# MiloszKrajewski/lz4net

Measured on AMD Instinct MI355X. Metric: uncompressed GB/s, batched 64KiB-block encode+decode: value = decode (known output size) per step over the whole resident batch; fast encode and LZ4HC encode of the same data in roofline_encode / roofline_hc, higher is better.
Workload: dtype u8

## Files before the change

lz4net_amd/csrc/lz4hip_decode_lane4.hpp:

```cpp
#pragma once
#include "lz4hip_common.hpp"
#include <type_traits>

#ifndef LZ4HIP_ITERATION_HOOK
#define LZ4HIP_ITERATION_HOOK(lane) ((void)0)
#endif
#ifndef LZ4HIP_STAT
#define LZ4HIP_STAT(slot, cond) ((void)0)
#endif
#ifdef LZ4HIP_SECTION_MARKERS
#define LZ4HIP_SECTION(name) asm volatile("; @@SECTION " name)
#else
#define LZ4HIP_SECTION(name) ((void)0)
#endif

namespace lz4hip {

#ifndef LZ4HIP_DEC4_FLUSH_RECS
#define LZ4HIP_DEC4_FLUSH_RECS 0
#endif
#ifndef LZ4HIP_DEC4_DUAL_STORE
#define LZ4HIP_DEC4_DUAL_STORE 2
#endif
constexpr unsigned lane4_lds_bytes(int ring_bytes) { return 64u * (unsigned)ring_bytes + 16u * 32u; }

struct NoNext {
    static constexpr bool kPersistent = false;
    LZ4HIP_DEVICE bool operator()(int, const uint8_t*&, int&, uint8_t*&, int&) const { return false; }
};

enum L4Kind { kK4None = 0, kK4Near = 1, kK4Far = 2, kK4Lit = 3, kK4Zero = 4 };
enum L4Flag { kF4Final = 1, kF4Err = 2, kF4Header = 4 };

template <bool KNOWN, int R, int P, int FU, int FS, int FE = 1, int IE = 1, int POL = 0, class NEXT = NoNext, int WAVES = 1>
LZ4HIP_DEVICE int lane4_decode_block(unsigned char* lds, int lane, bool active, const uint8_t* src, int iend,
                                     uint8_t* dst, int oend, NEXT next = NEXT(), int wave = 0)
{
    static_assert(WAVES == 1 || WAVES == 4, "one or four wavefronts per workgroup");
    constexpr uint32_t kRow = 256u * (uint32_t)WAVES;
    static_assert(R >= 128 && R % 16 == 0 && R <= 1008, "ring: a multiple of 16 bytes, 128 .. 1008");
    static_assert(P == 32 || P == 64, "input piece: 32 or 64 bytes");
    static_assert(FU == 64 || (FU == 128 && R >= 192), "flush unit: 64 bytes, or 128 with a ring of at least 192");
    static_assert(FS == 1 || FS == 2, "one or two flush store instructions per iteration");
    static_assert(FE == 1 || FE == 2, "the flush runs in every iteration or in every second one");
    static_assert(IE == 1 || (IE == 2 && FE == 2), "input requests in every iteration, or alternating with the flush");
    constexpr int RW = R / 4;
    constexpr bool RPOW2 = (RW & (RW - 1)) == 0;
    constexpr uint32_t kRingBytes = (uint32_t)RW * kRow;
    constexpr uint32_t kLdsBytes = lane4_lds_bytes(R) * (uint32_t)WAVES;
    constexpr bool LS = (POL & 16) != 0;
    constexpr int kDual = (POL & 32) ? 0 : (LZ4HIP_DEC4_DUAL_STORE);
    static_assert(!LS || P == 32, "sector input feeds 32-byte pieces");
    constexpr int SK = LS ? 64 : P;
    constexpr int NW = 4 + P / 4, NL = LS ? 4 : P / 16;
    constexpr int HPR = FU / 16, RECS_PER_STORE = 64 / HPR;
    constexpr int kFlushRecs = (LZ4HIP_DEC4_FLUSH_RECS) ? (LZ4HIP_DEC4_FLUSH_RECS) : FS * RECS_PER_STORE;
    constexpr bool kLineNoWrap = R % 64 == 0;
    constexpr int kNearMax = R - 20;
    unsigned char* const frec_base = lds + kRingBytes + (uint32_t)wave * 256u;
    auto frec = [&](int i) -> Aligned16* {
        if (kFlushRecs <= 16) return (Aligned16*)(frec_base + (uint32_t)i * 16u);
        return (Aligned16*)(frec_base + (uint32_t)(i >> 4) * kRow + (uint32_t)(i & 15) * 16u);
    };
    const uint32_t lane4 = (uint32_t)(wave * 64 + lane) << 2;

    auto ring_add = [](uint32_t a, uint32_t rows256) -> uint32_t {
        const uint32_t t = a + rows256;
        if (RPOW2) return t & (kRingBytes - 1u);
        const uint32_t u = t - kRingBytes;
        return u < t ? u : t;
    };
#define L4_RING(a) (*(uint32_t*)(lds + (a)))
#define L4_PHASE_SEL(p_) wv::alignbyte(0x07060504u, 0x03020100u, (uint32_t)(p_) & 3u)

    int skew = 0, in_total = 0;
    uint64_t src_al = 0;
    uint32_t out_limit = 0;
    int ip = 0;
    uint32_t W[NW];
    wv::u32x4 L[NL];
    int wb = -16;
    int lvalid = 0;
    int pend_a = 0, pend_b = 0;
    int op = 0, fl = 0;
    uint32_t oa = lane4;
    int kind = kK4None, rem = 0, off = 8;
    int gready = 0;
    int pv = 0, p_ll = 0, p_st = 0, p_ml = 0, p_off = 0, p_flags = 0, p_res = 0;
    uint32_t p_l0 = 0, p_l1 = 0, p_l2 = 0;
    int hdr = 0;
    uint32_t token = 0;
    int final_seen = 0, final_run = 0, result = 0, done = 0;
    int exhausted = 0;
    wv::u32x4 fa = { 0, 0, 0, 0 }, fb = { 0, 0, 0, 0 };
#if defined(LZ4HIP_DEC4_BALLAST_VALU) || defined(LZ4HIP_DEC4_BALLAST_LDS)
    uint32_t ballast = 0;
#endif
#pragma unroll
    for (int j = 0; j < NW; j++) W[j] = 0;
#pragma unroll
    for (int j = 0; j < NL; j++) L[j] = wv::u32x4{ 0, 0, 0, 0 };
    auto start_block = [&](bool act) {
        skew = (int)((uint64_t)src & (uint64_t)(SK - 1));
        src_al = (uint64_t)src - (uint64_t)skew;
        in_total = iend > 0 ? (int)(((int64_t)skew + iend + P - 1) & ~(int64_t)(P - 1)) : 0;
        out_limit = oend > kLastLiterals ? (uint32_t)(oend - kLastLiterals) : 0u;
        ip = 0; wb = -16 - P; lvalid = 0; pend_a = 0; pend_b = 0; op = 0; fl = 0; oa = lane4;
        kind = kK4None; rem = 0; off = 8; gready = 0;
        pv = 0; p_ll = 0; p_st = 0; p_ml = 0; p_off = 0; p_flags = 0; p_res = 0; hdr = 0; token = 0;
        final_seen = 0; final_run = 0; result = 0; done = 0;
        if (!act || (!KNOWN && iend == 0)) { done = 1; final_seen = 1; }
    };
    start_block(active);

#define L4_STORE2(OFF_, v_) do { const uint32_t w_ = (v_); wv::lds_store_drop<OFF_>(lds, kLdsBytes, oa, w_); wv::lds_store_drop<OFF_>(lds, kLdsBytes, ob_, w_); } while (0)
#define L4_APPEND(d0_, d1_, d2_, d3_, n_, FOUR_)                                                         \
    do {                                                                                                \
        const uint32_t sb_ = (uint32_t)op & 3u;                                                         \
        const uint32_t s_ = wv::alignbyte(0x08070605u, 0x04030201u, sb_ ^ 3u);                          \
        wv::lds_mskor(&L4_RING(oa), 0xFFFFFFFFu << (8u * sb_), wv::perm(d0_, 0u, s_));                  \
        if (kDual) {                                                                                    \
                                                    \
            const uint32_t ob_ = oa - kRingBytes;                                                       \
            const uint32_t w1_ = wv::perm(d1_, d0_, s_), w2_ = wv::perm(d2_, d1_, s_);                  \
            if (kDual == 2) {                                         \
                wv::lds_store2_rows_drop<1 * WAVES, 2 * WAVES>(lds, kLdsBytes, oa, w1_, w2_);           \
                wv::lds_store2_rows_drop<1 * WAVES, 2 * WAVES>(lds, kLdsBytes, ob_, w1_, w2_);          \
                if (FOUR_) {                                                                            \
                    const uint32_t w3_ = wv::perm(d3_, d2_, s_), w4_ = wv::perm(0u, d3_, s_);           \
                    wv::lds_store2_rows_drop<3 * WAVES, 4 * WAVES>(lds, kLdsBytes, oa, w3_, w4_);       \
                    wv::lds_store2_rows_drop<3 * WAVES, 4 * WAVES>(lds, kLdsBytes, ob_, w3_, w4_);      \
                } else {                                                                                \
                    L4_STORE2(3 * kRow, wv::perm(0u, d2_, s_));                                         \
                }                                                                                       \
            } else {                                                                                    \
                L4_STORE2(kRow, w1_);                                                                   \
                L4_STORE2(2 * kRow, w2_);                                                               \
                if (FOUR_) {                                                                            \
                    L4_STORE2(3 * kRow, wv::perm(d3_, d2_, s_));                                        \
                    L4_STORE2(4 * kRow, wv::perm(0u, d3_, s_));                                         \
                } else {                                                                                \
                    L4_STORE2(3 * kRow, wv::perm(0u, d2_, s_));                                         \
                }                                                                                       \
            }                                                                                           \
        } else {                                                                                        \
            const uint32_t a1_ = ring_add(oa, kRow), a2_ = ring_add(oa, 2 * kRow), a3_ = ring_add(oa, 3 * kRow); \
            L4_RING(a1_) = wv::perm(d1_, d0_, s_);                                                      \
            L4_RING(a2_) = wv::perm(d2_, d1_, s_);                                                      \
            if (FOUR_) {                                                                                \
                L4_RING(a3_) = wv::perm(d3_, d2_, s_);                                                  \
                L4_RING(ring_add(oa, 4 * kRow)) = wv::perm(0u, d3_, s_);                                \
            } else {                                                                                    \
                L4_RING(a3_) = wv::perm(0u, d2_, s_);                                                   \
            }                                                                                           \
        }                                                                                               \
        oa = ring_add(oa, (((sb_ + (uint32_t)(n_)) << 6) & 0x700u) * (uint32_t)WAVES);                  \
        op += (n_);                                                                                     \
    } while (0)

    auto iteration = [&](auto flush_tag, wv::u32x4& ldF, wv::u32x4& usF, int& ld_pend, int& us_pend) __attribute__((always_inline)) -> bool {
        constexpr bool FLUSH = decltype(flush_tag)::value;
        constexpr bool INPUT = IE == 1 || !FLUSH;
        constexpr int kVm = (FLUSH ? FS : 0) + 1 + (INPUT ? NL : 0);
        LZ4HIP_ITERATION_HOOK(lane);
        LZ4HIP_SECTION("T1a window refill");
        int d = ip + skew - wb;
        {
            const bool no_more = wb + 16 + P >= in_total;
            const bool cross = (d >= P) & ((lvalid != 0) | no_more);
            const wv::mask_t cm = wv::cond(d >= P) & (wv::cond(lvalid != 0) | wv::cond(no_more));
#pragma unroll
            for (int j = 0; j < 4; j++) W[j] = wv::sel(cm, W[P / 4 + j], W[j]);
            if constexpr (LS) {
                const bool hi_half = ((wb + 16 + P) & 32) != 0;
                const wv::mask_t hm = wv::cond(((wb + 16 + P) & 32) != 0);
#pragma unroll
                for (int j = 0; j < 2; j++) {
                    W[4 + 4 * j] = wv::sel(cm, wv::sel(hm, L[2 + j].x, L[j].x), W[4 + 4 * j]); W[5 + 4 * j] = wv::sel(cm, wv::sel(hm, L[2 + j].y, L[j].y), W[5 + 4 * j]);
                    W[6 + 4 * j] = wv::sel(cm, wv::sel(hm, L[2 + j].z, L[j].z), W[6 + 4 * j]); W[7 + 4 * j] = wv::sel(cm, wv::sel(hm, L[2 + j].w, L[j].w), W[7 + 4 * j]);
                }
                lvalid = (cross & hi_half) ? 0 : lvalid;
            } else {
#pragma unroll
                for (int j = 0; j < NL; j++) {
                    W[4 + 4 * j] = wv::sel(cm, L[j].x, W[4 + 4 * j]); W[5 + 4 * j] = wv::sel(cm, L[j].y, W[5 + 4 * j]);
                    W[6 + 4 * j] = wv::sel(cm, L[j].z, W[6 + 4 * j]); W[7 + 4 * j] = wv::sel(cm, L[j].w, W[7 + 4 * j]);
                }
                lvalid = cross ? 0 : lvalid;
            }
            wb += cross ? P : 0;
            d -= cross ? P : 0;
        }
        LZ4HIP_SECTION("T1b cursor view (select tree + rotation)");
        const bool staged16 = d < P;
        LZ4HIP_STAT(0, true); LZ4HIP_STAT(1, done == 0); LZ4HIP_STAT(2, (done == 0) & !staged16);
        uint32_t x0, x1, x2, x3;
        {
            const uint32_t k = (uint32_t)d >> 2;
            uint32_t t[NW];
#pragma unroll
            for (int j = 0; j < NW; j++) t[j] = W[j];
            int n = NW;
#pragma unroll
            for (int sh = P / 8; sh >= 1; sh >>= 1) {
                const wv::mask_t m = wv::cond((k & (uint32_t)sh) != 0u);
                n -= sh;
#pragma unroll
                for (int j = 0; j < NW; j++)
                    if (j < n) t[j] = wv::sel(m, t[j + sh], t[j]);
            }
            const uint32_t sx = L4_PHASE_SEL(d);
            x0 = wv::perm(t[1], t[0], sx); x1 = wv::perm(t[2], t[1], sx); x2 = wv::perm(t[3], t[2], sx); x3 = wv::perm(t[4], t[3], sx);
        }
        LZ4HIP_SECTION("T1c near-match source rows");
        uint32_t v0, v1, v2, v3;
        {
            const uint32_t offn = kind == kK4Near ? (uint32_t)off : 4u;
            const uint32_t back = (((offn + 3u - ((uint32_t)op & 3u)) << 6) & ~0xFFu) * (uint32_t)WAVES;
            uint32_t sa;
            if (RPOW2) sa = (oa - back) & (kRingBytes - 1u);
            else { const uint32_t t = oa - back, u = t + kRingBytes; sa = u < t ? u : t; }
            const uint32_t r0 = L4_RING(sa), r1 = L4_RING(ring_add(sa, kRow)), r2 = L4_RING(ring_add(sa, 2 * kRow)),
                           r3 = L4_RING(ring_add(sa, 3 * kRow)), r4 = L4_RING(ring_add(sa, 4 * kRow));
            const uint32_t sr = L4_PHASE_SEL((uint32_t)op - offn);
            v0 = wv::perm(r1, r0, sr); v1 = wv::perm(r2, r1, sr); v2 = wv::perm(r3, r2, sr); v3 = wv::perm(r4, r3, sr);
        }

        LZ4HIP_SECTION("T2 cooperative flush");
        if constexpr (FLUSH) {
            const bool need = (done == 0) & (op - fl >= FU);
            const uint64_t needy = wv::ballot(need);
            const int cnt_all = wv::popc64(needy);
            const bool go = cnt_all != 0;
            int cnt = 0;
            bool mine = false;
            if (go) {
                cnt = cnt_all < kFlushRecs ? cnt_all : kFlushRecs;
                const int frank = wv::rank_below(needy);
                mine = need & (frank < kFlushRecs);
                if (mine) {
                    const uint64_t dp = (uint64_t)dst;
                    *frec(frank) = Aligned16{ { ring_add(oa, kRingBytes - ((((uint32_t)(op - fl)) << 6) & ~0xFFu) * (uint32_t)WAVES), (uint32_t)fl, (uint32_t)dp, (uint32_t)(dp >> 32) } };
                }
                wv::mem_sync();
            }
            const int sub = lane % HPR;
#pragma unroll
            for (int base = 0; base < FS * RECS_PER_STORE; base += RECS_PER_STORE) {
                const int idx = base + lane / HPR;
                const bool act = idx < cnt;
                const wv::mask_t act_m = wv::cond(idx < cnt);
                uint64_t g = 0;
                uint32_t q0 = 0, q1 = 0, q2 = 0, q3 = 0;
                if (act) {
                    const Aligned16 r = *frec(idx);
                    g = ((uint64_t)r.w[2] | ((uint64_t)r.w[3] << 32)) + (uint64_t)(r.w[1] + 16u * (uint32_t)sub);
                    const uint32_t b0 = ring_add(r.w[0], 4u * kRow * (uint32_t)sub);
                    if (kLineNoWrap) { q0 = L4_RING(b0); q1 = L4_RING(b0 + kRow); q2 = L4_RING(b0 + 2 * kRow); q3 = L4_RING(b0 + 3 * kRow); }
                    else { q0 = L4_RING(b0); q1 = L4_RING(ring_add(b0, kRow)); q2 = L4_RING(ring_add(b0, 2 * kRow)); q3 = L4_RING(ring_add(b0, 3 * kRow)); }
                }
                wv::vm_store16_mask(act_m, g, q0, q1, q2, q3);
            }
            LZ4HIP_STAT(3, need); LZ4HIP_STAT(4, need & !mine);
            if (go) {
                wv::mem_sync();
                fl += mine ? FU : 0;
            }
        }
        LZ4HIP_SECTION("T3 chunk size");
        const bool room = op - fl <= R - 46;
        const bool near = kind == kK4Near, lit = kind == kK4Lit;
        const bool can = room & (rem > 0) & !((kind == kK4Far) & (gready == 0)) & !(lit & !staged16);
        const int stride = (near & (off < 16)) ? off : 16;
        int n = can ? (rem < stride ? rem : stride) : 0;
        n = ((kind == kK4Zero) & (n > 8)) ? 8 : n;
        LZ4HIP_STAT(5, (done == 0) & (rem > 0)); LZ4HIP_STAT(6, (done == 0) & (rem > 0) & (n == 0)); LZ4HIP_STAT(7, (done == 0) & (rem > 0) & !room);
        LZ4HIP_STAT(8, (done == 0) & (rem > 0) & (kind == kK4Far) & (gready == 0)); LZ4HIP_STAT(9, (done == 0) & (rem > n));
        const int rem_after = rem - n;
        const int op_end = op + rem;

        LZ4HIP_SECTION("T4 parse ahead");
        const bool may_parse = (pv == 0) & (final_seen == 0) & !(lit & (rem > 0)) & staged16;
        LZ4HIP_STAT(10, may_parse); LZ4HIP_STAT(11, (done == 0) & (pv != 0));
        if (may_parse) {
            const uint32_t tok = hdr ? token : (x0 & 255u);
            const uint32_t t4 = tok >> 4, b1 = (x0 >> 8) & 255u, mlc = tok & 15u;
            const bool e1 = (hdr == 0) & (t4 == 15u), e2 = mlc == 15u;
            const int ll = hdr ? 0 : (int)t4 + (e1 ? (int)b1 : 0);
            const bool in_win = (hdr != 0) | (t4 <= 11u);
            const int o = hdr ? 0 : 1 + (int)t4;
            uint32_t ot;
            {
                const uint32_t q = (uint32_t)o >> 2;
                const wv::mask_t m1 = wv::cond((q & 1u) != 0u), m2 = wv::cond((q & 2u) != 0u);
                const uint32_t lo = wv::sel(m2, wv::sel(m1, x3, x2), wv::sel(m1, x1, x0));
                const uint32_t hi = wv::sel(m2, x3, wv::sel(m1, x2, x1));
                ot = wv::alignbyte(hi, lo, (uint32_t)o & 3u);
            }
            const int vo = (int)(ot & 0xFFFFu);
            const uint32_t extb = (ot >> 16) & 255u;
            const int ml = (int)mlc + kMinMatch + (e2 ? (int)extb : 0);
            const int lit_end = op_end + ll;
            const int p_after = ip + o + 2;
            bool trap = (ip + 16 > iend) | (e1 & (b1 == 255u)) | (ip + 1 + (e1 ? 1 : 0) + ll > iend);
            trap |= in_win & ((e2 & (extb == 255u)) | (vo > lit_end) | ((uint32_t)lit_end + (uint32_t)ml > out_limit));
            if (KNOWN) trap |= (hdr == 0) & (lit_end > oend - 8);
            else       trap |= ((hdr == 0) & ((lit_end > oend - kMfLimit) | (ip + 1 + (e1 ? 1 : 0) + ll > iend - 8))) | (in_win & e2 & !(p_after < iend - (kLastLiterals + 1)));
            p_l0 = wv::alignbyte(x1, x0, 1); p_l1 = wv::alignbyte(x2, x1, 1); p_l2 = wv::alignbyte(x3, x2, 1);
            token = tok;
            p_ll = in_win ? ll : 0;
            p_st = in_win ? 0 : ll;
            p_ml = in_win ? ml : 0;
            p_off = vo;
            p_flags = in_win ? 0 : (int)kF4Header;
            const int ip_fast = in_win ? p_after + (e2 ? 1 : 0) : ip + 1 + (e1 ? 1 : 0);
            if (trap) {
                LZ4HIP_SECTION("T4x byte-wise parser (trap)");
                int err = 0, pos = ip;
                if (!hdr) {
                    const uint32_t tk = ip < iend ? src[ip] : 0u;
                    int l = (int)(tk >> 4);
                    pos = ip + 1;
                    if (l == 15) {
                        uint32_t b = 255;
                        if (KNOWN) { do { b = pos < iend ? src[pos] : 0u; pos++; l += (int)b; if (l > (1 << 30)) { err = -pos; l = 0; break; } } while (b == 255); }
                        else       { while (pos < iend && b == 255) { b = src[pos]; pos++; l += (int)b; l = l > (1 << 30) ? (1 << 30) : l; } }
                    }
                    token = tk;
                    const int le = (int)((int64_t)op_end + l > 0x7FFFFFFF ? 0x7FFFFFFF : op_end + l);
                    const bool last = KNOWN ? (le > oend - 8) : ((le > oend - kMfLimit) | (pos + l > iend - 8));
                    p_ll = 0; p_st = l; p_ml = 0; p_off = 8;
                    if (last) {
                        if (KNOWN) { if (err == 0 && (le != oend || pos + l > iend)) err = -pos; }
                        else       { if (le > oend || pos + l != iend) err = -pos; }
                        p_flags = kF4Final;
                        p_res = KNOWN ? pos + l : le;
                        final_seen = 1;
                    } else {
                        if (KNOWN && err == 0 && pos + l > iend) err = -pos;
                        p_flags = kF4Header;
                    }
                    ip = pos;
                } else {
                    int p = ip;
                    const int o_ = (int)((p < iend ? src[p] : 0u) | ((p + 1 < iend ? src[p + 1] : 0u) << 8));
                    p += 2;
                    int m = (int)(token & 15u);
                    if (m == 15) {
                        if (KNOWN) {
                            uint32_t b;
                            while ((b = (p < iend ? src[p] : 0u)) == 255) { m += 255; p++; if (m > (1 << 30)) { err = -p; break; } }
                            m += (int)b; p++;
                        } else {
                            while (p < iend - (kLastLiterals + 1)) { const uint32_t b = src[p]; p++; m += (int)b; m = m > (1 << 30) ? (1 << 30) : m; if (b != 255) break; }
                        }
                    }
                    m += kMinMatch;
                    if (err != 0) {}
                    else if (op_end - o_ < 0) err = -(ip + 2);
                    else if ((int64_t)op_end + m > (int64_t)oend - kLastLiterals) err = -p;
                    p_ll = 0; p_st = 0; p_ml = m; p_off = o_; p_flags = 0;
                    ip = p;
                    hdr = 0;
                }
                if (err != 0) { p_flags = kF4Err; p_res = err; }
                hdr = (p_flags & kF4Header) ? 1 : 0;
            } else {
                ip = ip_fast;
                hdr = in_win ? 0 : 1;
            }
            LZ4HIP_SECTION("T4 parse ahead");
            pv = 1;
        }

        LZ4HIP_SECTION("T5 far fetch");
        {
            const wv::mask_t m_rem0 = wv::cond(rem_after == 0);
            const wv::mask_t f_cont = wv::cond(kind == kK4Far) & ~m_rem0;
            const wv::mask_t f_first = m_rem0 & wv::cond(op - fl <= R - 46) & wv::cond(pv != 0) & wv::cond(p_ml != 0) & wv::cond(p_flags == 0) & wv::cond(p_off > kNearMax);
            const int f_pos = (int)wv::sel(f_cont, (uint32_t)(op + n - off), (uint32_t)(op_end + p_ll - p_off));
            const wv::mask_t f_want = f_cont | f_first;
            const wv::mask_t f_do = f_want & wv::cond(f_pos + 16 <= fl);
            wv::vm_load16_mask<POL & 3>(f_do, (uint64_t)dst + (uint64_t)(uint32_t)f_pos, ldF);
            gready = (int)wv::sel(f_do, 1u, 0u);
            LZ4HIP_STAT(15, gready != 0); LZ4HIP_STAT(16, wv::sel(f_want & ~f_do, 1u, 0u) != 0u);
        }

        LZ4HIP_SECTION("T6 input request");
        if constexpr (INPUT) {
            const int lpos = wb + 16 + P;
            const wv::mask_t req = wv::cond((done | lvalid | us_pend) == 0) & wv::cond(lpos < in_total);
            const uint64_t g = src_al + (uint64_t)(uint32_t)lpos;
            wv::vm_load16_mask_off<(POL >> 2) & 3, 0>(req, g, L[0]);
            wv::vm_load16_mask_off<(POL >> 2) & 3, 16>(req, g, L[1]);
            if constexpr (NL == 4) {
                wv::vm_load16_mask_off<(POL >> 2) & 3, 32>(req, g, L[2]);
                wv::vm_load16_mask_off<(POL >> 2) & 3, 48>(req, g, L[3]);
            }
            ld_pend = (int)wv::sel(req, 1u, 0u);
        } else {
            ld_pend = 0;
        }

        LZ4HIP_SECTION("B1 wait");
        wv::vm_wait_list<kVm>(usF, L);
        lvalid = us_pend ? 1 : lvalid;
        us_pend = 0;

#if defined(LZ4HIP_DEC4_BALLAST_VALU) || defined(LZ4HIP_DEC4_BALLAST_LDS)
#ifdef LZ4HIP_DEC4_BALLAST_VALU
#pragma unroll
        for (int bi = 0; bi < LZ4HIP_DEC4_BALLAST_VALU; bi++) asm volatile("v_add_u32 %0, %0, %1" : "+v"(ballast) : "v"(lane4));
#endif
#ifdef LZ4HIP_DEC4_BALLAST_LDS
#pragma unroll
        for (int bi = 0; bi < LZ4HIP_DEC4_BALLAST_LDS; bi++) wv::lds_store_drop<0>(lds, kLdsBytes, 0x80000000u + lane4, ballast);
#endif
#endif
        LZ4HIP_SECTION("B3 chunk append");
        {
            const bool far_src = kind == kK4Far;
            v0 = lit ? x0 : (far_src ? usF.x : v0);
            v1 = lit ? x1 : (far_src ? usF.y : v1);
            v2 = lit ? x2 : (far_src ? usF.z : v2);
            v3 = lit ? x3 : (far_src ? usF.w : v3);
            if ((kind == kK4Zero) & (n > 0)) {
                uint64_t acc = 0;
                for (int b = 0; b < n; b++) acc |= (uint64_t)dst[op + b] << (8 * b);
                v0 = (uint32_t)acc; v1 = (uint32_t)(acc >> 32);
            }
            ip += lit ? n : 0;
            L4_APPEND(v0, v1, v2, v3, n, true);
            rem = rem_after;
            off = (near & (off < 16) & (n > 0)) ? off * 2 : off;
            kind = rem == 0 ? (int)kK4None : kind;
        }

        LZ4HIP_SECTION("B4 promote + literal append");
        {
            const bool promote = (rem == 0) & (pv != 0) & room;
            LZ4HIP_STAT(12, promote); LZ4HIP_STAT(13, (done == 0) & (rem == 0) & (pv != 0) & !room); LZ4HIP_STAT(14, (done == 0) & (rem == 0) & (pv == 0));
            const bool perr = promote & ((p_flags & kF4Err) != 0);
            const bool pgo = promote & !perr;
            L4_APPEND(p_l0, p_l1, p_l2, 0u, pgo ? p_ll : 0, false);
            if (perr) {
                done = 1; final_seen = 1; final_run = 0; result = p_res;
            }
            if (pgo) {
                const bool streamed = p_st > 0;
                rem = streamed ? p_st : p_ml;
                off = streamed ? off : p_off;
                kind = streamed ? (int)kK4Lit : (p_ml == 0 ? (int)kK4None : (p_off == 0 ? (int)kK4Zero : (p_off <= kNearMax ? (int)kK4Near : (int)kK4Far)));
                final_run = (p_flags & kF4Final) ? 1 : final_run;
                result = (p_flags & kF4Final) ? p_res : result;
            }
            pv = promote ? 0 : pv;
        }

        LZ4HIP_SECTION("B5 end of block + loop");
        if (final_run && rem == 0 && !pv && !done) {
            uint32_t qa = ring_add(oa, kRingBytes - ((((uint32_t)(op - fl)) << 6) & ~0xFFu) * (uint32_t)WAVES);
            while (op - fl >= 4) { const uint32_t qd = L4_RING(qa); __builtin_memcpy(dst + fl, &qd, 4); fl += 4; qa = ring_add(qa, kRow); }
            if (fl < op) {
                const uint32_t qd = L4_RING(qa);
                for (int b = 0; fl + b < op; b++) dst[fl + b] = (uint8_t)(qd >> (8 * b));
            }
            done = 1;
        }
        return !wv::any(done == 0);
    };

    for (;;) {
        if (!std::remove_reference<NEXT>::type::kPersistent) {
            if (iteration(std::true_type{}, fa, fb, pend_a, pend_b)) break;
            if (iteration(std::integral_constant<bool, FE == 1>{}, fb, fa, pend_b, pend_a)) break;
        } else {
            (void)iteration(std::true_type{}, fa, fb, pend_a, pend_b);
            (void)iteration(std::integral_constant<bool, FE == 1>{}, fb, fa, pend_b, pend_a);
            const bool fin = (done != 0) & (exhausted == 0);
            if (wv::any(fin)) {
                if (fin) {
                    if (next(result, src, iend, dst, oend)) start_block(true);
                    else exhausted = 1;
                }
                if (!wv::any(exhausted == 0)) break;
            }
        }
    }
    return result;
#undef L4_RING
#undef L4_PHASE_SEL
#undef L4_APPEND
#undef L4_STORE2
}

__global__ void __launch_bounds__(256) count_selected_kernel(Batch b, int filter, unsigned* count)
{
    unsigned mine = 0;
    for (int64_t blk = (int64_t)blockIdx.x * 256 + threadIdx.x; blk < b.n_blocks; blk += (int64_t)gridDim.x * 256)
        mine += block_selected(filter, batch_src_len(b, blk), batch_dst_cap(b, blk)) ? 1u : 0u;
    const unsigned total = wv::scan_add(mine);
    if ((threadIdx.x & 63u) == 63u && total) atomicAdd(count, total);
}
LZ4HIP_DEVICE bool lane4_gate_open(const unsigned* gate, int gate_mode, unsigned threshold)
{
    if (gate_mode == 0) return true;
    const unsigned c = wv::uniform(*gate);
    return gate_mode == 1 ? c >= threshold : c < threshold;
}

__global__ void __launch_bounds__(64) lds_drop_probe_kernel(unsigned* errors, int rounds)
{
    constexpr uint32_t kBytes = lane4_lds_bytes(192), kRing = 64u * 192u, kWords = kBytes / 4u;
    LZ4HIP_STATIC_LDS(lds, kBytes);
    uint32_t* const s = (uint32_t*)lds;
    const uint32_t lane = threadIdx.x, tag = 0x9E3779B9u * (blockIdx.x + 1u);
    for (uint32_t i = lane; i < kWords; i += 64u) s[i] = tag ^ i;
    wv::block_sync();
    for (int r = 0; r < rounds; r++) {
        const uint32_t junk = 0xDEAD0000u | (uint32_t)r;
        const uint32_t last = kRing - 256u + lane * 4u;
        const uint32_t own = tag ^ (last >> 2);
        wv::lds_store2_rows_drop<0, 3>(lds, kBytes, last, own, junk);
        wv::lds_store2_rows_drop<3, 4>(lds, kBytes, last, junk, junk);
        wv::lds_store_drop<1024>(lds, kBytes, last, junk);
        wv::lds_store_drop<768>(lds, kBytes, kBytes - 256u + lane * 4u, junk);
        const uint32_t neg = lane * 4u - kRing;
        wv::lds_store2_rows_drop<1, 2>(lds, kBytes, neg, junk, junk);
        wv::lds_store2_rows_drop<3, 4>(lds, kBytes, neg + 2048u, junk, junk);
        wv::lds_store_drop<768>(lds, kBytes, neg, junk);
        wv::lds_store2_rows_drop<0, 48>(lds, kBytes, neg, junk, tag ^ lane);
        wv::mem_sync();
#if defined(__HIP_DEVICE_COMPILE__)
        __builtin_amdgcn_s_sleep(8);
#endif
    }
    wv::block_sync();
    unsigned bad = 0;
    for (uint32_t i = lane; i < kWords; i += 64u) bad += s[i] != (tag ^ i) ? 1u : 0u;
    if (bad) atomicAdd(errors, bad);
}

template <bool KNOWN, int R, int P, int FU, int FS, int FE = 1, int IE = 1, int POL = 0>
__global__ void __launch_bounds__(64) decode_lane4_kernel(Batch b, int filter, const unsigned* gate = nullptr, int gate_mode = 0, unsigned threshold = 0)
{
    LZ4HIP_STATIC_LDS(lds, lane4_lds_bytes(R));
    if (!lane4_gate_open(gate, gate_mode, threshold)) return;
    const int lane = (int)threadIdx.x;
    const int64_t blk = (int64_t)blockIdx.x * 64 + lane;
    bool active = blk < b.n_blocks;
    int src_len = 0, out_size = 0;
    if (active) {
        src_len = batch_src_len(b, blk); out_size = batch_dst_cap(b, blk);
        active = block_selected(filter, src_len, out_size);
    }
    if (!wv::any(active)) return;
    const uint8_t* src = active ? batch_src(b, blk) : nullptr;
    uint8_t* dst = active ? batch_dst(b, blk) : nullptr;
    const int r = lane4_decode_block<KNOWN, R, P, FU, FS, FE, IE, POL>(lds, lane, active, src, src_len, dst, out_size);
    if (active) b.result[blk] = r;
}

template <bool KNOWN, int R, int P, int FU, int FS, int FE = 1, int IE = 1, int POL = 0>
__global__ void __launch_bounds__(256) decode_lane4_wg4_kernel(Batch b, int filter)
{
    LZ4HIP_STATIC_LDS(lds_all, 4u * lane4_lds_bytes(R));
    const int lane = (int)(threadIdx.x & 63u);
    const int w = wv::wave_in_block();
    const int64_t blk = ((int64_t)blockIdx.x * 4 + w) * 64 + lane;
    bool active = blk < b.n_blocks;
    int src_len = 0, out_size = 0;
    if (active) {
        src_len = batch_src_len(b, blk); out_size = batch_dst_cap(b, blk);
        active = block_selected(filter, src_len, out_size);
    }
    if (!wv::any(active)) return;
    const uint8_t* src = active ? batch_src(b, blk) : nullptr;
    uint8_t* dst = active ? batch_dst(b, blk) : nullptr;
    const int r = lane4_decode_block<KNOWN, R, P, FU, FS, FE, IE, POL, NoNext, 4>(lds_all, lane, active, src, src_len, dst, out_size, NoNext(), w);
    if (active) b.result[blk] = r;
}

struct PullNext {
    static constexpr bool kPersistent = true;
    const Batch* b; int filter; unsigned long long* counter; int64_t cur;
    LZ4HIP_DEVICE bool operator()(int r, const uint8_t*& src, int& iend, uint8_t*& dst, int& oend)
    {
        if (cur >= 0) b->result[cur] = r;
        for (;;) {
            const int64_t blk = (int64_t)atomicAdd(counter, 1ull);
            if (blk >= b->n_blocks) { cur = -1; return false; }
            const int sl = batch_src_len(*b, blk), oc = batch_dst_cap(*b, blk);
            if (!block_selected(filter, sl, oc)) continue;
            cur = blk; src = batch_src(*b, blk); iend = sl; dst = batch_dst(*b, blk); oend = oc;
            return true;
        }
    }
};

template <bool KNOWN, int R, int P, int FU, int FS, int FE = 1, int IE = 1, int POL = 0>
__global__ void __launch_bounds__(64) decode_lane4_persistent_kernel(Batch b, int filter, unsigned long long* counter, const unsigned* gate = nullptr,
                                                                     int gate_mode = 0, unsigned threshold = 0)
{
    LZ4HIP_STATIC_LDS(lds, lane4_lds_bytes(R));
    if (!lane4_gate_open(gate, gate_mode, threshold)) return;
    const int lane = (int)threadIdx.x;
    PullNext next{ &b, filter, counter, -1 };
    const uint8_t* src = nullptr; uint8_t* dst = nullptr; int src_len = 0, out_size = 0;
    const bool active = next(0, src, src_len, dst, out_size);
    if (!wv::any(active)) return;
    (void)lane4_decode_block<KNOWN, R, P, FU, FS, FE, IE, POL, PullNext&>(lds, lane, active, src, src_len, dst, out_size, next);
}

}
```

Measured before the change: 1037.

## Split cooperative flush into record, row-read and deferred store phases

The cooperative flush is split into three phases: record publishing and record reads move to the top of the iteration, ring row reads stay in place, and the global stores are deferred until after parse-ahead. This spreads the LDS reads and global stores across independent work so their latency can overlap with window refill and parsing. The fl advance now happens before the ring rows are read, which changes ordering relative to the room and flush-eligibility checks. More values stay live across the iteration (FS records, addresses and 4 words each), which raises register pressure. Optional section-state and report hooks are added for profiling.

```diff
diff --git a/lz4net_amd/csrc/lz4hip_decode_lane4.hpp b/lz4net_amd/csrc/lz4hip_decode_lane4.hpp
--- a/lz4net_amd/csrc/lz4hip_decode_lane4.hpp
+++ b/lz4net_amd/csrc/lz4hip_decode_lane4.hpp
@@ -8,10 +8,15 @@
 #ifndef LZ4HIP_STAT
 #define LZ4HIP_STAT(slot, cond) ((void)0)
 #endif
-#ifdef LZ4HIP_SECTION_MARKERS
+#if defined(LZ4HIP_SECTION)
+#elif defined(LZ4HIP_SECTION_MARKERS)
 #define LZ4HIP_SECTION(name) asm volatile("; @@SECTION " name)
 #else
 #define LZ4HIP_SECTION(name) ((void)0)
+#endif
+#ifndef LZ4HIP_SECTION_STATE
+#define LZ4HIP_SECTION_STATE() ((void)0)
+#define LZ4HIP_SECTION_REPORT() ((void)0)
 #endif
 
 namespace lz4hip {
@@ -63,6 +68,7 @@
         return (Aligned16*)(frec_base + (uint32_t)(i >> 4) * kRow + (uint32_t)(i & 15) * 16u);
     };
     const uint32_t lane4 = (uint32_t)(wave * 64 + lane) << 2;
+    LZ4HIP_SECTION_STATE();
 
     auto ring_add = [](uint32_t a, uint32_t rows256) -> uint32_t {
         const uint32_t t = a + rows256;
@@ -163,6 +169,39 @@
         constexpr bool INPUT = IE == 1 || !FLUSH;
         constexpr int kVm = (FLUSH ? FS : 0) + 1 + (INPUT ? NL : 0);
         LZ4HIP_ITERATION_HOOK(lane);
+        LZ4HIP_SECTION("T2a flush records");
+        bool f_go = false, f_act[FS] = {};
+        wv::mask_t f_act_m[FS] = {};
+        Aligned16 f_rec[FS] = {};
+        uint64_t f_g[FS] = {};
+        uint32_t f_q[FS][4] = {};
+        if constexpr (FLUSH) {
+            const bool need = (done == 0) & (op - fl >= FU);
+            const uint64_t needy = wv::ballot(need);
+            const int cnt_all = wv::popc64(needy);
+            f_go = cnt_all != 0;
+            int cnt = 0;
+            bool mine = false;
+            if (f_go) {
+                cnt = cnt_all < kFlushRecs ? cnt_all : kFlushRecs;
+                const int frank = wv::rank_below(needy);
+                mine = need & (frank < kFlushRecs);
+                if (mine) {
+                    const uint64_t dp = (uint64_t)dst;
+                    *frec(frank) = Aligned16{ { ring_add(oa, kRingBytes - ((((uint32_t)(op - fl)) << 6) & ~0xFFu) * (uint32_t)WAVES), (uint32_t)fl, (uint32_t)dp, (uint32_t)(dp >> 32) } };
+                }
+                wv::mem_sync();
+                fl += mine ? FU : 0;
+            }
+#pragma unroll
+            for (int k = 0; k < FS; k++) {
+                const int idx = k * RECS_PER_STORE + lane / HPR;
+                f_act[k] = idx < cnt;
+                f_act_m[k] = wv::cond(idx < cnt);
+                if (f_act[k]) f_rec[k] = *frec(idx);
+            }
+            LZ4HIP_STAT(3, need); LZ4HIP_STAT(4, need & !mine);
+        }
         LZ4HIP_SECTION("T1a window refill");
         int d = ip + skew - wb;
         {
@@ -226,46 +265,19 @@
             v0 = wv::perm(r1, r0, sr); v1 = wv::perm(r2, r1, sr); v2 = wv::perm(r3, r2, sr); v3 = wv::perm(r4, r3, sr);
         }
 
-        LZ4HIP_SECTION("T2 cooperative flush");
+        LZ4HIP_SECTION("T2b flush rows");
         if constexpr (FLUSH) {
-            const bool need = (done == 0) & (op - fl >= FU);
-            const uint64_t needy = wv::ballot(need);
-            const int cnt_all = wv::popc64(needy);
-            const bool go = cnt_all != 0;
-            int cnt = 0;
-            bool mine = false;
-            if (go) {
-                cnt = cnt_all < kFlushRecs ? cnt_all : kFlushRecs;
-                const int frank = wv::rank_below(needy);
-                mine = need & (frank < kFlushRecs);
-                if (mine) {
-                    const uint64_t dp = (uint64_t)dst;
-                    *frec(frank) = Aligned16{ { ring_add(oa, kRingBytes - ((((uint32_t)(op - fl)) << 6) & ~0xFFu) * (uint32_t)WAVES), (uint32_t)fl, (uint32_t)dp, (uint32_t)(dp >> 32) } };
+#pragma unroll
+            for (int k = 0; k < FS; k++) {
+                if (f_act[k]) {
+                    const Aligned16 r = f_rec[k];
+                    f_g[k] = ((uint64_t)r.w[2] | ((uint64_t)r.w[3] << 32)) + (uint64_t)(r.w[1] + 16u * (uint32_t)(lane % HPR));
+                    const uint32_t b0 = ring_add(r.w[0], 4u * kRow * (uint32_t)(lane % HPR));
+                    if (kLineNoWrap) { f_q[k][0] = L4_RING(b0); f_q[k][1] = L4_RING(b0 + kRow); f_q[k][2] = L4_RING(b0 + 2 * kRow); f_q[k][3] = L4_RING(b0 + 3 * kRow); }
+                    else { f_q[k][0] = L4_RING(b0); f_q[k][1] = L4_RING(ring_add(b0, kRow)); f_q[k][2] = L4_RING(ring_add(b0, 2 * kRow)); f_q[k][3] = L4_RING(ring_add(b0, 3 * kRow)); }
                 }
-                wv::mem_sync();
-            }
-            const int sub = lane % HPR;
-#pragma unroll
-            for (int base = 0; base < FS * RECS_PER_STORE; base += RECS_PER_STORE) {
-                const int idx = base + lane / HPR;
-                const bool act = idx < cnt;
-                const wv::mask_t act_m = wv::cond(idx < cnt);
-                uint64_t g = 0;
-                uint32_t q0 = 0, q1 = 0, q2 = 0, q3 = 0;
-                if (act) {
-                    const Aligned16 r = *frec(idx);
-                    g = ((uint64_t)r.w[2] | ((uint64_t)r.w[3] << 32)) + (uint64_t)(r.w[1] + 16u * (uint32_t)sub);
-                    const uint32_t b0 = ring_add(r.w[0], 4u * kRow * (uint32_t)sub);
-                    if (kLineNoWrap) { q0 = L4_RING(b0); q1 = L4_RING(b0 + kRow); q2 = L4_RING(b0 + 2 * kRow); q3 = L4_RING(b0 + 3 * kRow); }
-                    else { q0 = L4_RING(b0); q1 = L4_RING(ring_add(b0, kRow)); q2 = L4_RING(ring_add(b0, 2 * kRow)); q3 = L4_RING(ring_add(b0, 3 * kRow)); }
-                }
-                wv::vm_store16_mask(act_m, g, q0, q1, q2, q3);
-            }
-            LZ4HIP_STAT(3, need); LZ4HIP_STAT(4, need & !mine);
-            if (go) {
-                wv::mem_sync();
-                fl += mine ? FU : 0;
-            }
+            }
+            if (f_go) wv::mem_sync();
         }
         LZ4HIP_SECTION("T3 chunk size");
         const bool room = op - fl <= R - 46;
@@ -373,6 +385,12 @@
             pv = 1;
         }
 
+        LZ4HIP_SECTION("T2c flush stores");
+        if constexpr (FLUSH) {
+#pragma unroll
+            for (int k = 0; k < FS; k++) wv::vm_store16_mask(f_act_m[k], f_g[k], f_q[k][0], f_q[k][1], f_q[k][2], f_q[k][3]);
+        }
+
         LZ4HIP_SECTION("T5 far fetch");
         {
             const wv::mask_t m_rem0 = wv::cond(rem_after == 0);
@@ -487,6 +505,7 @@
             }
         }
     }
+    LZ4HIP_SECTION_REPORT();
     return result;
 #undef L4_RING
 #undef L4_PHASE_SEL
```

After: 1035. No clear change (-0.2%).
